# yuliakot/snark-verifier-axiom

Hardware: AMD Instinct MI355X
Metric: BN254 G1 MSM points/sec at 2^20 + KZG pairings/sec; 1/2/4/8 GPU (higher is better)
Workload: dtype u32 (254-bit Montgomery field: bucket chain 9x29-bit limbs, elsewhere 8x32-bit)

## Files before the change

### snark-verifier-axiom_amd/csrc/curve29.hpp

```cpp
#pragma once
#include "field29.hpp"

namespace sv {
namespace r29 {

struct Xyzz {
  F X, Y, ZZ, ZZZ;
};

SV29_HD F one() {
  F r;
  constexpr uint32_t O[L] = {0x157ccc21u, 0x141c2758u, 0x185230d3u, 0x14c0419u, 0xaa36fb9u,
                             0x1d4240ceu, 0x11d54c07u, 0x52ac7a8u,  0x00dc836u};
#pragma unroll
  for (int i = 0; i < L; i++) r.v[i] = O[i];
  return r;
}
SV29_HD Xyzz identity() { return {zero(), zero(), zero(), zero()}; }
SV29_HD bool is_identity(const Xyzz& p) { return is_zero(p.ZZ); }

SV29_HD Xyzz madd(const Xyzz& p, const F& x2, const F& y2, bool neg) {
  if (is_identity(p)) return {x2, neg ? sub<2>(zero(), y2) : y2, one(), one()};
  F Pd = sub<8>(mul(x2, p.ZZ), p.X);
  F Rd = sub_sgn<4>(mul(y2, p.ZZZ), neg, p.Y);
  F X = p.X, Y = p.Y, ZZ = p.ZZ, ZZZ = p.ZZZ;
  bool dbl = false;
  if (is_zero_mod_p_10p(Pd)) {
    if (!is_zero_mod_p_6p(Rd)) return identity();
    const F x2s = sqr(x2), ys = neg ? sub<2>(zero(), y2) : y2;
    Pd = add(ys, ys);
    Rd = add(add(x2s, x2s), x2s);
    X = x2, Y = ys, ZZ = one(), ZZZ = one();
    dbl = true;
  }
  const F PP = sqr(Pd), PPP = mul(Pd, PP), Q = mul(X, PP), R2 = sqr(Rd);
  const F X3 = sub_2c<6>(R2, dbl ? zero() : PPP, Q);
  const F Y3 = mul_sum2(Rd, sub<8>(Q, X3), Y, sub<2>(zero(), PPP));
  return {X3, Y3, mul(ZZ, PP), mul(ZZZ, PPP)};
}
SV29_HD Xyzz madd(const Xyzz& p, const F& x2, const F& y2) { return madd(p, x2, y2, false); }

SV29_HD F neg_one() {
  F r;
  constexpr uint32_t O[L] = {0x3003126u, 0xce8395eu, 0x420727bu, 0x1891eb7u, 0xae269bfu,
                             0x598fff2u, 0xed19539u, 0x9315e8bu, 0x229c18u};
#pragma unroll
  for (int i = 0; i < L; i++) r.v[i] = O[i];
  return r;
}
SV29_HD Xyzz start(const F& x2, const F& y2, bool neg) { return {x2, y2, one(), neg ? neg_one() : one()}; }
SV29_HD Xyzz madd_live(const Xyzz& p, const F& x2, const F& y2, bool neg, int& special) {
  const F Pd = mul_sub<8>(x2, p.ZZ, p.X);
  const F Rd = sub_sgn<4>(mul(y2, p.ZZZ), neg, p.Y);
  if (is_zero_mod_p_10p(Pd)) special = is_zero_mod_p_6p(Rd) ? 2 : 1;
  const F PP = sqr(Pd), PPP = mul(Pd, PP), Q = mul(p.X, PP);
  const F X3 = sqr_sub2c<6>(Rd, PPP, Q);
  const F Y3 = mul_sum2(Rd, sub<8>(Q, X3), p.Y, sub<2>(zero(), PPP));
  return {X3, Y3, mul(p.ZZ, PP), mul(p.ZZZ, PPP)};
}
SV29_HD Xyzz dbl_start(const F& x2, const F& y2, bool neg) {
  const F ys = neg ? sub<2>(zero(), y2) : y2;
  const F x2s = sqr(x2);
  const F Pd = add(ys, ys);
  const F Rd = add(add(x2s, x2s), x2s);
  const F PP = sqr(Pd), PPP = mul(Pd, PP), Q = mul(x2, PP);
  const F X3 = sqr_sub2c<6>(Rd, zero(), Q);
  const F Y3 = mul_sum2(Rd, sub<8>(Q, X3), ys, sub<2>(zero(), PPP));
  return {X3, Y3, PP, PPP};
}

template <bool kX4>
SV29_HD Xyzz add_t(const Xyzz& p, const Xyzz& q) {
  if (is_identity(p)) {
    if constexpr (kX4) return {csub<4>(q.X), q.Y, q.ZZ, q.ZZZ};
    else return q;
  }
  if (is_identity(q)) {
    if constexpr (kX4) return {csub<4>(p.X), p.Y, p.ZZ, p.ZZZ};
    else return p;
  }
  F U1 = mul(p.X, q.ZZ), S1 = mul(p.Y, q.ZZZ);
  F Pd = sub<2>(mul(q.X, p.ZZ), U1), Rd = sub<2>(mul(q.Y, p.ZZZ), S1);
  F qZZ = q.ZZ, qZZZ = q.ZZZ;
  bool dbl = false;
  if (is_zero_mod_p_6p(Pd)) {
    if (!is_zero_mod_p_6p(Rd)) return identity();
    const F x2 = sqr(p.X);
    Pd = add(p.Y, p.Y);
    Rd = add(add(x2, x2), x2);
    U1 = p.X, S1 = p.Y, qZZ = one(), qZZZ = one();
    dbl = true;
  }
  const F PP = sqr(Pd), PPP = mul(Pd, PP), Q = mul(U1, PP), R2 = sqr(Rd);
  const F X3 = csub<4>(sub<4>(dbl ? R2 : sub<2>(R2, PPP), add(Q, Q)));
  const F Y3 = mul_sum2(Rd, sub<4>(Q, X3), S1, sub<2>(zero(), PPP));
  return {X3, Y3, mul(mul(p.ZZ, qZZ), PP), mul(mul(p.ZZZ, qZZZ), PPP)};
}
SV29_HD Xyzz add(const Xyzz& p, const Xyzz& q) { return add_t<true>(p, q); }
SV29_HD Xyzz add_x8(const Xyzz& p, const Xyzz& q) { return add_t<false>(p, q); }

}
}
```

### snark-verifier-axiom_amd/csrc/field29.hpp

```cpp
#pragma once
#include <cstdint>

#if defined(__HIPCC__) || defined(__HIP__)
#include <hip/hip_runtime.h>
#define SV29_HD __host__ __device__ __forceinline__
#else
#define SV29_HD inline
#endif

namespace sv {
namespace r29 {

constexpr int L = 9;
constexpr uint32_t MASK = (1u << 29) - 1;

struct FqM29 {
  static constexpr uint32_t NP = 0x4866389u;
  SV29_HD static constexpr uint32_t kp(int k, int i) {
    constexpr uint32_t T[9][9] = {
        {0, 0, 0, 0, 0, 0, 0, 0, 0},
        {0x187cfd47u, 0x10460b6u, 0x1c72a34fu, 0x2d522d0u, 0x1585d978u, 0x2db40c0u, 0xa6e141u, 0xe5c2634u, 0x30644eu},
        {0x10f9fa8eu, 0x208c16du, 0x18e5469eu, 0x5aa45a1u, 0xb0bb2f0u, 0x5b68181u, 0x14dc282u, 0x1cb84c68u, 0x60c89cu},
        {0x976f7d5u, 0x30d2224u, 0x1557e9edu, 0x87f6872u, 0x918c68u, 0x891c242u, 0x1f4a3c3u, 0xb14729cu, 0x912cebu},
        {0x1f3f51cu, 0x41182dbu, 0x11ca8d3cu, 0xb548b43u, 0x161765e0u, 0xb6d0302u, 0x29b8504u, 0x197098d0u, 0xc19139u},
        {0x1a70f263u, 0x515e391u, 0xe3d308bu, 0xe29ae14u, 0xb9d3f58u, 0xe4843c3u, 0x3426645u, 0x7ccbf04u, 0xf1f588u},
        {0x12edefaau, 0x61a4448u, 0xaafd3dau, 0x10fed0e5u, 0x12318d0u, 0x11238484u, 0x3e94786u, 0x1628e538u, 0x12259d6u},
        {0xb6aecf1u, 0x71ea4ffu, 0x7227729u, 0x13d3f3b6u, 0x16a8f248u, 0x13fec544u, 0x49028c7u, 0x4850b6cu, 0x152be25u},
        {0x3e7ea38u, 0x82305b6u, 0x3951a78u, 0x16a91687u, 0xc2ecbc0u, 0x16da0605u, 0x5370a08u, 0x12e131a0u, 0x1832273u}};
    return T[k][i];
  }
};
struct FrM29 {
  static constexpr uint32_t NP = 0xfffffffu;
  SV29_HD static constexpr uint32_t kp(int k, int i) {
    constexpr uint32_t T[9][9] = {
        {0, 0, 0, 0, 0, 0, 0, 0, 0},
        {0x10000001u, 0x1f0fac9fu, 0xe5c2450u, 0x7d090f3u, 0x1585d283u, 0x2db40c0u, 0xa6e141u, 0xe5c2634u, 0x30644eu},
        {0x2u, 0x1e1f593fu, 0x1cb848a1u, 0xfa121e6u, 0xb0ba506u, 0x5b68181u, 0x14dc282u, 0x1cb84c68u, 0x60c89cu},
        {0x10000003u, 0x1d2f05deu, 0xb146cf2u, 0x1771b2dau, 0x917789u, 0x891c242u, 0x1f4a3c3u, 0xb14729cu, 0x912cebu},
        {0x4u, 0x1c3eb27eu, 0x19709143u, 0x1f4243cdu, 0x16174a0cu, 0xb6d0302u, 0x29b8504u, 0x197098d0u, 0xc19139u},
        {0x10000005u, 0x1b4e5f1du, 0x7ccb594u, 0x712d4c1u, 0xb9d1c90u, 0xe4843c3u, 0x3426645u, 0x7ccbf04u, 0xf1f588u},
        {0x6u, 0x1a5e0bbdu, 0x1628d9e5u, 0xee365b4u, 0x122ef13u, 0x11238484u, 0x3e94786u, 0x1628e538u, 0x12259d6u},
        {0x10000007u, 0x196db85cu, 0x484fe36u, 0x16b3f6a8u, 0x16a8c196u, 0x13fec544u, 0x49028c7u, 0x4850b6cu, 0x152be25u},
        {0x8u, 0x187d64fcu, 0x12e12287u, 0x1e84879bu, 0xc2e9419u, 0x16da0605u, 0x5370a08u, 0x12e131a0u, 0x1832273u}};
    return T[k][i];
  }
};

template <class M>
struct F29 {
  uint32_t v[L];
};
using F = F29<FqM29>;

template <class M = FqM29>
SV29_HD F29<M> zero() {
  F29<M> r;
#pragma unroll
  for (int i = 0; i < L; i++) r.v[i] = 0;
  return r;
}
template <int K, class M = FqM29>
SV29_HD F29<M> kp_f() {
  F29<M> r;
#pragma unroll
  for (int i = 0; i < L; i++) r.v[i] = M::kp(K, i);
  return r;
}

template <class M = FqM29>
SV29_HD F29<M> from_words(const uint32_t* w) {
  F29<M> r;
#pragma unroll
  for (int i = 0; i < L; i++) {
    const int bit = 29 * i, j = bit >> 5, s = bit & 31;
    uint32_t x = w[j] >> s;
    if (s > 3 && j + 1 < 8) x |= w[j + 1] << (32 - s);
    r.v[i] = x & MASK;
  }
  return r;
}
template <class M>
SV29_HD void to_words(const F29<M>& a, uint32_t* w) {
#pragma unroll
  for (int j = 0; j < 8; j++) {
    const int bit = 32 * j, i = bit / 29, s = bit % 29;
    uint32_t x = a.v[i] >> s;
    if (i + 1 < L) x |= a.v[i + 1] << (29 - s);
    if (s > 26 && i + 2 < L) x |= a.v[i + 2] << (58 - s);
    w[j] = x;
  }
}

SV29_HD uint64_t mad(uint32_t a, uint32_t b, uint64_t c) { return (uint64_t)a * b + c; }

#define SV29_REDUCE_COLUMN(k)                                          \
  {                                                                    \
    _Pragma("unroll") for (int i = 0; i < L; i++) {                    \
      const int j = (k) - i;                                           \
      if (i < (k) && j >= 1 && j < L) acc = mad(m[i], M::kp(1, j), acc); \
    }                                                                  \
    if ((k) < L) {                                                     \
      m[(k)] = ((uint32_t)acc * M::NP) & MASK;                         \
      acc = mad(m[(k)], M::kp(1, 0), acc);                             \
    } else {                                                           \
      t.v[(k) - L] = (uint32_t)acc & MASK;                             \
    }                                                                  \
    acc >>= 29;                                                        \
  }

template <class M>
SV29_HD F29<M> mul(const F29<M>& a, const F29<M>& b) {
  uint32_t m[L];
  F29<M> t;
  uint64_t acc = 0;
#pragma unroll
  for (int k = 0; k < 2 * L - 1; k++) {
#pragma unroll
    for (int i = 0; i < L; i++) {
      const int j = k - i;
      if (j >= 0 && j < L) acc = mad(a.v[i], b.v[j], acc);
    }
    SV29_REDUCE_COLUMN(k)
  }
  t.v[L - 1] = (uint32_t)acc;
  return t;
}

template <class M>
SV29_HD F29<M> sqr(const F29<M>& a) {
  uint32_t m[L], a2[L];
  F29<M> t;
#pragma unroll
  for (int i = 0; i < L; i++) a2[i] = a.v[i] << 1;
  uint64_t acc = 0;
#pragma unroll
  for (int k = 0; k < 2 * L - 1; k++) {
#pragma unroll
    for (int i = 0; i < L; i++) {
      const int j = k - i;
      if (j > i && j < L) acc = mad(a.v[i], a2[j], acc);
    }
    if ((k & 1) == 0 && k / 2 < L) acc = mad(a.v[k / 2], a.v[k / 2], acc);
    SV29_REDUCE_COLUMN(k)
  }
  t.v[L - 1] = (uint32_t)acc;
  return t;
}

template <class M>
SV29_HD F29<M> mul_sum2(const F29<M>& a0, const F29<M>& b0, const F29<M>& a1, const F29<M>& b1) {
  uint32_t m[L];
  F29<M> t;
  uint64_t acc = 0;
#pragma unroll
  for (int k = 0; k < 2 * L - 1; k++) {
#pragma unroll
    for (int i = 0; i < L; i++) {
      const int j = k - i;
      if (j >= 0 && j < L) {
        acc = mad(a0.v[i], b0.v[j], acc);
        acc = mad(a1.v[i], b1.v[j], acc);
      }
    }
    SV29_REDUCE_COLUMN(k)
  }
  t.v[L - 1] = (uint32_t)acc;
  return t;
}
template <class M>
SV29_HD F29<M> mul_sum3(const F29<M>& a0, const F29<M>& b0, const F29<M>& a1, const F29<M>& b1,
                        const F29<M>& a2, const F29<M>& b2) {
  uint32_t m[L];
  F29<M> t;
  uint64_t acc = 0;
#pragma unroll
  for (int k = 0; k < 2 * L - 1; k++) {
#pragma unroll
    for (int i = 0; i < L; i++) {
      const int j = k - i;
      if (j >= 0 && j < L) {
        acc = mad(a0.v[i], b0.v[j], acc);
        acc = mad(a1.v[i], b1.v[j], acc);
        acc = mad(a2.v[i], b2.v[j], acc);
      }
    }
    SV29_REDUCE_COLUMN(k)
  }
  t.v[L - 1] = (uint32_t)acc;
  return t;
}
template <class M>
SV29_HD F29<M> mul_add_hi(const F29<M>& a, const F29<M>& b, const uint32_t D[L]) {
  uint32_t m[L];
  F29<M> t;
  uint64_t acc = 0;
#pragma unroll
  for (int k = 0; k < 2 * L - 1; k++) {
    if (k >= L) acc += D[k - L];
#pragma unroll
    for (int i = 0; i < L; i++) {
      const int j = k - i;
      if (j >= 0 && j < L) acc = mad(a.v[i], b.v[j], acc);
    }
    SV29_REDUCE_COLUMN(k)
  }
  t.v[L - 1] = ((uint32_t)acc + D[L - 1]) & MASK;
  return t;
}
template <class M>
SV29_HD F29<M> sqr_add_hi(const F29<M>& a, const uint32_t D[L]) {
  uint32_t m[L], a2[L];
  F29<M> t;
#pragma unroll
  for (int i = 0; i < L; i++) a2[i] = a.v[i] << 1;
  uint64_t acc = 0;
#pragma unroll
  for (int k = 0; k < 2 * L - 1; k++) {
    if (k >= L) acc += D[k - L];
#pragma unroll
    for (int i = 0; i < L; i++) {
      const int j = k - i;
      if (j > i && j < L) acc = mad(a.v[i], a2[j], acc);
    }
    if ((k & 1) == 0 && k / 2 < L) acc = mad(a.v[k / 2], a.v[k / 2], acc);
    SV29_REDUCE_COLUMN(k)
  }
  t.v[L - 1] = ((uint32_t)acc + D[L - 1]) & MASK;
  return t;
}
#undef SV29_REDUCE_COLUMN

template <int K, class M>
SV29_HD F29<M> mul_sub(const F29<M>& a, const F29<M>& b, const F29<M>& c) {
  uint32_t D[L];
#pragma unroll
  for (int i = 0; i < L; i++) D[i] = (M::kp(K, i) + (1u << 29) - (i > 0 ? 1u : 0u)) - c.v[i];
  return mul_add_hi(a, b, D);
}
template <int K, class M>
SV29_HD F29<M> sqr_sub2c(const F29<M>& a, const F29<M>& b, const F29<M>& c) {
  uint32_t D[L];
#pragma unroll
  for (int i = 0; i < L; i++) D[i] = (M::kp(K, i) + (3u << 29) - (i > 0 ? 3u : 0u)) - (b.v[i] + (c.v[i] << 1));
  return sqr_add_hi(a, D);
}

template <class M>
SV29_HD F29<M> mul_ilp(const F29<M>& a, const F29<M>& b) {
  uint64_t c[2 * L - 1];
#pragma unroll
  for (int k = 0; k < 2 * L - 1; k++) c[k] = 0;
#pragma unroll
  for (int i = 0; i < L; i++)
#pragma unroll
    for (int j = 0; j < L; j++) c[i + j] = mad(a.v[i], b.v[j], c[i + j]);
#pragma unroll
  for (int k = 0; k < L; k++) {
    const uint32_t m = ((uint32_t)c[k] * M::NP) & MASK;
    c[k] = mad(m, M::kp(1, 0), c[k]);
    c[k + 1] += c[k] >> 29;
#pragma unroll
    for (int j = 1; j < L; j++) c[k + j] = mad(m, M::kp(1, j), c[k + j]);
  }
  F29<M> t;
  uint64_t carry = 0;
#pragma unroll
  for (int i = 0; i < L - 1; i++) {
    const uint64_t x = c[L + i] + carry;
    t.v[i] = (uint32_t)x & MASK;
    carry = x >> 29;
  }
  t.v[L - 1] = (uint32_t)carry;
  return t;
}

template <int K, class M>
SV29_HD F29<M> sub(const F29<M>& a, const F29<M>& b) {
  F29<M> r;
  int32_t c = 0;
#pragma unroll
  for (int i = 0; i < L; i++) {
    const int32_t x = (int32_t)(a.v[i] + M::kp(K, i)) - (int32_t)b.v[i] + c;
    c = x >> 29;
    r.v[i] = (uint32_t)x & MASK;
  }
  return r;
}

template <class M>
SV29_HD F29<M> add(const F29<M>& a, const F29<M>& b) {
  F29<M> r;
  uint32_t c = 0;
#pragma unroll
  for (int i = 0; i < L; i++) {
    const uint32_t x = a.v[i] + b.v[i] + c;
    c = x >> 29;
    r.v[i] = x & MASK;
  }
  return r;
}

template <int K, class M>
SV29_HD F29<M> sub_2c(const F29<M>& a, const F29<M>& b, const F29<M>& c) {
  F29<M> r;
  int32_t cy = 0;
#pragma unroll
  for (int i = 0; i < L; i++) {
    const int32_t x = (int32_t)(a.v[i] + M::kp(K, i)) - (int32_t)b.v[i] - 2 * (int32_t)c.v[i] + cy;
    cy = x >> 29;
    r.v[i] = (uint32_t)x & MASK;
  }
  return r;
}

template <int K, class M>
SV29_HD F29<M> sub_sgn(const F29<M>& a, bool neg, const F29<M>& b) {
  F29<M> r;
  int32_t cy = 0;
  const uint32_t sgn = neg ? 0xffffffffu : 1u;
#pragma unroll
  for (int i = 0; i < L; i++) {
    const int32_t x = (int32_t)(a.v[i] * sgn) + (int32_t)M::kp(K, i) - (int32_t)b.v[i] + cy;
    cy = x >> 29;
    r.v[i] = (uint32_t)x & MASK;
  }
  return r;
}

template <int K, class M>
SV29_HD F29<M> csub(const F29<M>& a) {
  F29<M> d;
  int32_t c = 0;
#pragma unroll
  for (int i = 0; i < L; i++) {
    const int32_t x = (int32_t)a.v[i] - (int32_t)M::kp(K, i) + c;
    c = x >> 29;
    d.v[i] = (uint32_t)x & MASK;
  }
  return c < 0 ? a : d;
}

template <class M>
SV29_HD bool eq(const F29<M>& a, const F29<M>& b) {
  uint32_t x = 0;
#pragma unroll
  for (int i = 0; i < L; i++) x |= a.v[i] ^ b.v[i];
  return x == 0;
}
template <class M>
SV29_HD bool is_zero(const F29<M>& a) {
  uint32_t x = 0;
#pragma unroll
  for (int i = 0; i < L; i++) x |= a.v[i];
  return x == 0;
}

SV29_HD bool is_zero_mod_p_16p(const F& a) {
  constexpr float kInvPTop = 3.1531752142655023e-07f;
  const uint32_t k = (uint32_t)((float)a.v[L - 1] * kInvPTop + 0.5f);
  if (a.v[0] != ((k * FqM29::kp(1, 0)) & MASK)) return false;
  return is_zero(csub<1>(csub<2>(csub<4>(csub<8>(a)))));
}
SV29_HD bool is_zero_mod_p_6p(const F& a) { return is_zero_mod_p_16p(a); }
SV29_HD bool is_zero_mod_p_10p(const F& a) { return is_zero_mod_p_16p(a); }

template <class M = FqM29>
SV29_HD F29<M> to_r29(const uint32_t* w) {
  F29<M> r;
#pragma unroll
  for (int i = 0; i < L; i++) {
    if (i == 0) {
      r.v[0] = (w[0] << 5) & MASK;
      continue;
    }
    const int bit = 29 * i - 5, j = bit >> 5, s = bit & 31;
    uint32_t x = w[j] >> s;
    if (s > 3 && j + 1 < 8) x |= w[j + 1] << (32 - s);
    r.v[i] = x & MASK;
  }
  const uint32_t q = (uint32_t)(((uint64_t)r.v[L - 1] * (0xffffffffull / (M::kp(1, L - 1) + 1))) >> 32);
  int64_t c = 0;
#pragma unroll
  for (int i = 0; i < L; i++) {
    const int64_t x = (int64_t)r.v[i] - (int64_t)q * M::kp(1, i) + c;
    c = x >> 29;
    r.v[i] = (uint32_t)x & MASK;
  }
  return csub<2>(r);
}
template <class M>
SV29_HD void to_r32(const F29<M>& a, uint32_t* w) {
  const uint32_t m = (a.v[0] * M::NP) & 31;
  F29<M> t;
  uint64_t c = 0;
#pragma unroll
  for (int i = 0; i < L; i++) {
    c += (uint64_t)m * M::kp(1, i) + a.v[i];
    t.v[i] = (uint32_t)c & MASK;
    c >>= 29;
  }
  F29<M> d;
#pragma unroll
  for (int i = 0; i < L; i++) d.v[i] = (t.v[i] >> 5) | ((i + 1 < L ? t.v[i + 1] : (uint32_t)c) << 24 & MASK);
  to_words(csub<1>(d), w);
}

}
}
```

### snark-verifier-axiom_amd/csrc/msm.hip

```cpp
#include <hip/hip_runtime.h>

#include <algorithm>
#include <chrono>
#include <cmath>
#include <cstdio>
#include <cstdlib>
#include <cstring>
#include <atomic>
#include <functional>
#include <string>
#include <thread>
#include <type_traits>
#include <vector>

#include "curve.hpp"
#include "curve29.hpp"
#include "glv.hpp"
#include "host_ec.hpp"
#include "msm.hpp"
#include "msm_batch.hpp"
#include "quad.hpp"
#include "runtime.hpp"

namespace sv {
// ... 120 lines not shown
  reinterpret_cast<uint4*>(out + i)[1] = make_uint4(r.x.v[4], r.x.v[5], r.x.v[6], r.x.v[7]);
  reinterpret_cast<uint4*>(out + i)[2] = make_uint4(r.y.v[0], r.y.v[1], r.y.v[2], r.y.v[3]);
  reinterpret_cast<uint4*>(out + i)[3] = make_uint4(r.y.v[4], r.y.v[5], r.y.v[6], r.y.v[7]);
}

template <int C, int NB>
__host__ __device__ constexpr int num_windows() { return (NB + C - 1) / C; }
template <int C, int NB = 255, class F>
__device__ __forceinline__ void for_each_digit(const Fr& s, F&& f) {
  constexpr int W = num_windows<C, NB>();
  uint32_t carry = 0;
  const uint32_t half = 1u << (C - 1);
  const uint32_t mask = (1u << C) - 1;
#pragma unroll
  for (int w = 0; w < W; w++) {
    const int pos = w * C;
    const int limb = pos >> 5, off = pos & 31;
    const uint32_t lo = limb < 8 ? s.v[limb] : 0;
    const uint32_t hi = (limb + 1) < 8 ? s.v[limb + 1] : 0;
    uint32_t bits = off ? ((lo >> off) | (hi << (32 - off))) : lo;
    bits = (bits & mask) + carry;
    if (bits > half) {
      f(w, (1u << C) - bits, 1u);
      carry = 1;
    } else {
      f(w, bits, 0u);
      carry = 0;
    }
  }
}

__device__ __forceinline__ Fr scalar_in(const uint4 q0, const uint4 q1, int mont_in, uint32_t* __restrict__ err) {
  Fr s;
  s.v[0] = q0.x; s.v[1] = q0.y; s.v[2] = q0.z; s.v[3] = q0.w;
  s.v[4] = q1.x; s.v[5] = q1.y; s.v[6] = q1.z; s.v[7] = q1.w;
  if (err && !s.is_reduced()) atomicOr(err, 2u);
  return mont_in ? fe_from_mont(s) : s;
}
__device__ __forceinline__ Fr load_scalar(const Fr* __restrict__ scalars, uint32_t i, int mont_in,
                                          uint32_t* __restrict__ err) {
  const uint4* p = reinterpret_cast<const uint4*>(scalars + i);
  const uint4 q0 = p[0], q1 = p[1];
  Fr s;
  s.v[0] = q0.x; s.v[1] = q0.y; s.v[2] = q0.z; s.v[3] = q0.w;
  s.v[4] = q1.x; s.v[5] = q1.y; s.v[6] = q1.z; s.v[7] = q1.w;
  if (err && !s.is_reduced()) atomicOr(err, 2u);
  return mont_in ? fe_from_mont(s) : s;
}

template <int C, bool GLV>
struct Digits {
  static constexpr int NB = GLV ? 128 : 255;
  static constexpr int W = num_windows<C, NB>();
  static constexpr int EP = GLV ? 2 * W : W;
  uint32_t h[GLV ? 2 : 1][GLV ? 4 : 8];
  uint32_t sgn[GLV ? 2 : 1];
  __device__ __forceinline__ void load(const Fr* __restrict__ scalars, uint32_t i, int mont_in,
                                       uint32_t* __restrict__ err) {
    from(load_scalar(scalars, i, mont_in, err));
  }
  __device__ __forceinline__ void from(const Fr& s) {
    if constexpr (GLV) {
      uint32_t h1[4], h2[4];
      glv_split(s.v, h1, h2);
#pragma unroll
      for (int k = 0; k < 4; k++) h[0][k] = h1[k], h[1][k] = h2[k];
#pragma unroll
      for (int q = 0; q < 2; q++) {
        sgn[q] = h[q][3] >> 31;
        h[q][3] &= 0x7fffffffu;
      }
    } else {
#pragma unroll
      for (int k = 0; k < 8; k++) h[0][k] = s.v[k];
      sgn[0] = 0;
    }
  }
  __device__ __forceinline__ void store(uint4* __restrict__ hv, uint32_t i) const {
    if constexpr (GLV) {
      hv[2 * i] = make_uint4(h[0][0], h[0][1], h[0][2], h[0][3] | (sgn[0] << 31));
      hv[2 * i + 1] = make_uint4(h[1][0], h[1][1], h[1][2], h[1][3] | (sgn[1] << 31));
    } else {
      hv[2 * i] = make_uint4(h[0][0], h[0][1], h[0][2], h[0][3]);
      hv[2 * i + 1] = make_uint4(h[0][4], h[0][5], h[0][6], h[0][7]);
    }
  }
  __device__ __forceinline__ void load_stored(const uint4* __restrict__ hv, uint32_t i) {
    const uint4 a = hv[2 * i], b = hv[2 * i + 1];
    if constexpr (GLV) {
      h[0][0] = a.x; h[0][1] = a.y; h[0][2] = a.z; h[0][3] = a.w & 0x7fffffffu;
      h[1][0] = b.x; h[1][1] = b.y; h[1][2] = b.z; h[1][3] = b.w & 0x7fffffffu;
      sgn[0] = a.w >> 31;
      sgn[1] = b.w >> 31;
    } else {
      h[0][0] = a.x; h[0][1] = a.y; h[0][2] = a.z; h[0][3] = a.w;
      h[0][4] = b.x; h[0][5] = b.y; h[0][6] = b.z; h[0][7] = b.w;
      sgn[0] = 0;
    }
  }
  template <class F>
  __device__ __forceinline__ void each(F&& f) const {
#pragma unroll
    for (int q = 0; q < (GLV ? 2 : 1); q++) {
      Fr s;
      if constexpr (GLV) {
#pragma unroll
        for (int k = 0; k < 4; k++) s.v[k] = h[q][k], s.v[4 + k] = 0u;
      } else {
#pragma unroll
        for (int k = 0; k < 8; k++) s.v[k] = h[0][k];
      }
      const uint32_t sg = sgn[q];
      for_each_digit<C, NB>(s, [&](int w, uint32_t mag, uint32_t neg) { f(w, mag, neg ^ sg, (uint32_t)q); });
    }
  }
};

__device__ __forceinline__ void glv_phix(const G1Aff* __restrict__ bases, uint32_t i, uint4* __restrict__ phix,
                                         int phi64, uint32_t* __restrict__ err) {
  const uint4* b = reinterpret_cast<const uint4*>(bases + i);
  Fq x, beta;
  const uint4 x0 = b[0], x1 = b[1];
  x.v[0] = x0.x; x.v[1] = x0.y; x.v[2] = x0.z; x.v[3] = x0.w;
  x.v[4] = x1.x; x.v[5] = x1.y; x.v[6] = x1.z; x.v[7] = x1.w;
#pragma unroll
  for (int j = 0; j < 8; j++) beta.v[j] = GLV_BETA_MONT[j];
  const Fq bx = x * beta;
  uint4* o = phix + (phi64 ? 4 : 2) * i;
  o[0] = make_uint4(bx.v[0], bx.v[1], bx.v[2], bx.v[3]);
  o[1] = make_uint4(bx.v[4], bx.v[5], bx.v[6], bx.v[7]);
  if (phi64 || err) {
    const uint4 y0 = b[2], y1 = b[3];
    if (phi64) {
      o[2] = y0;
      o[3] = y1;
    }
    if (err) {
      Fq y;
      y.v[0] = y0.x; y.v[1] = y0.y; y.v[2] = y0.z; y.v[3] = y0.w;
      y.v[4] = y1.x; y.v[5] = y1.y; y.v[6] = y1.z; y.v[7] = y1.w;
      if (!x.is_reduced() || !y.is_reduced()) atomicOr(err, 1u);
    }
  }
}

__global__ void k_glv_phix(const G1Aff* __restrict__ bases, uint32_t n, uint4* __restrict__ phix, int phi64,
                           uint32_t* __restrict__ err) {
  const uint32_t i = blockIdx.x * blockDim.x + threadIdx.x;
  if (i < n) glv_phix(bases, i, phix, phi64, err);
}

static constexpr int kPhiVtab = 2;
static constexpr int kVtabRec = 9;
__device__ __forceinline__ void st_rec29(uint2* o, const r29::F& x, const r29::F& y) {
  o[0] = make_uint2(x.v[0], x.v[1]);
  o[1] = make_uint2(x.v[2], x.v[3]);
  o[2] = make_uint2(x.v[4], x.v[5]);
  o[3] = make_uint2(x.v[6], x.v[7]);
  o[4] = make_uint2(x.v[8], y.v[0]);
  o[5] = make_uint2(y.v[1], y.v[2]);
  o[6] = make_uint2(y.v[3], y.v[4]);
  o[7] = make_uint2(y.v[5], y.v[6]);
  o[8] = make_uint2(y.v[7], y.v[8]);
}
__device__ __forceinline__ void ld_rec29(const uint2* __restrict__ o, r29::F& x, r29::F& y) {
  uint2 q[kVtabRec];
#pragma unroll
  for (int k = 0; k < kVtabRec; k++) q[k] = o[k];
  x.v[0] = q[0].x, x.v[1] = q[0].y, x.v[2] = q[1].x, x.v[3] = q[1].y, x.v[4] = q[2].x, x.v[5] = q[2].y;
  x.v[6] = q[3].x, x.v[7] = q[3].y, x.v[8] = q[4].x;
  y.v[0] = q[4].y, y.v[1] = q[5].x, y.v[2] = q[5].y, y.v[3] = q[6].x, y.v[4] = q[6].y, y.v[5] = q[7].x;
  y.v[6] = q[7].y, y.v[7] = q[8].x, y.v[8] = q[8].y;
}
__device__ __forceinline__ void vtab_put_pt(const G1Aff& a, uint32_t i, uint4* __restrict__ vtab, uint32_t nsplit,
                                            bool glv, uint32_t* __restrict__ err) {
  if (err && (!a.x.is_reduced() || !a.y.is_reduced())) atomicOr(err, 1u);
  const r29::F y = r29::to_r29(a.y.v), x = r29::to_r29(a.x.v);
  uint2* t = reinterpret_cast<uint2*>(vtab);
  st_rec29(t + kVtabRec * (size_t)i, x, y);
  if (glv) {
    constexpr uint32_t kBeta29[r29::L] = {0xa337995u, 0x158d1d23u, 0x189c9b98u, 0x12fa4e45u, 0x185faadcu,
                                         0x176f16du, 0xeed93bau,  0x14291140u, 0xc0afeu};
    r29::F beta;
#pragma unroll
    for (int j = 0; j < r29::L; j++) beta.v[j] = kBeta29[j];
    st_rec29(t + kVtabRec * ((size_t)nsplit + i), r29::mul(x, beta), y);
  }
}
__device__ __forceinline__ void vtab_put(const G1Aff* __restrict__ bases, uint32_t i, uint4* __restrict__ vtab,
                                         uint32_t nsplit, bool glv, uint32_t* __restrict__ err) {
  vtab_put_pt(load_aff(bases, i), i, vtab, nsplit, glv, err);
}
__global__ void k_vtab(const G1Aff* __restrict__ bases, uint32_t n, uint4* __restrict__ vtab, int glv,
                       uint32_t* __restrict__ err) {
  const uint32_t i = blockIdx.x * blockDim.x + threadIdx.x;
  if (i < n) vtab_put(bases, i, vtab, n, glv != 0, err);
}

__global__ void __launch_bounds__(kBlock) k_resident_prepare(const G1Aff* in, G1Aff* out, uint32_t n, int mont_in,
                                                             uint4* __restrict__ vtab, uint32_t* __restrict__ err) {
  const uint32_t i = blockIdx.x * blockDim.x + threadIdx.x;
  if (i >= n) return;
  G1Aff a;
  {
    const uint4* p = reinterpret_cast<const uint4*>(in + i);
    const uint4 q0 = p[0], q1 = p[1], q2 = p[2], q3 = p[3];
    a.x.v[0] = q0.x; a.x.v[1] = q0.y; a.x.v[2] = q0.z; a.x.v[3] = q0.w;
    a.x.v[4] = q1.x; a.x.v[5] = q1.y; a.x.v[6] = q1.z; a.x.v[7] = q1.w;
    a.y.v[0] = q2.x; a.y.v[1] = q2.y; a.y.v[2] = q2.z; a.y.v[3] = q2.w;
    a.y.v[4] = q3.x; a.y.v[5] = q3.y; a.y.v[6] = q3.z; a.y.v[7] = q3.w;
  }
  if (!a.x.is_reduced() || !a.y.is_reduced()) {
    atomicOr(err, 1u);
    a.x = Fq::zero();
    a.y = Fq::zero();
  }
  if (!mont_in && !a.is_identity()) {
    a.x = fe_to_mont(a.x);
    a.y = fe_to_mont(a.y);
  }
  uint4* o = reinterpret_cast<uint4*>(out + i);
  o[0] = make_uint4(a.x.v[0], a.x.v[1], a.x.v[2], a.x.v[3]);
  o[1] = make_uint4(a.x.v[4], a.x.v[5], a.x.v[6], a.x.v[7]);
  o[2] = make_uint4(a.y.v[0], a.y.v[1], a.y.v[2], a.y.v[3]);
  o[3] = make_uint4(a.y.v[4], a.y.v[5], a.y.v[6], a.y.v[7]);
  vtab_put_pt(a, i, vtab, n, true, nullptr);
}

__global__ void k_check_bases(const G1Aff* __restrict__ bases, uint32_t n, uint32_t* __restrict__ err) {
  const uint32_t i = blockIdx.x * blockDim.x + threadIdx.x;
  if (i >= n) return;
  const G1Aff a = load_aff(bases, i);
  if (!a.x.is_reduced() || !a.y.is_reduced()) atomicOr(err, 1u);
}

__host__ __device__ constexpr int ceil_log2(int x) { return x <= 1 ? 0 : 1 + ceil_log2((x + 1) / 2); }

template <int N>
__device__ __forceinline__ uint32_t block_excl_scan(uint32_t* x, uint32_t* part) {
  constexpr int PER = (N + kBlock - 1) / kBlock;
  const int tid = threadIdx.x;
  uint32_t loc[PER];
  uint32_t sum = 0;
#pragma unroll
  for (int j = 0; j < PER; j++) {
    const int k = tid * PER + j;
    loc[j] = k < N ? x[k] : 0u;
    sum += loc[j];
  }
  part[tid] = sum;
  __syncthreads();
  for (int off = 1; off < kBlock; off <<= 1) {
    const uint32_t u = tid >= off ? part[tid - off] : 0u;
    __syncthreads();
    part[tid] += u;
    __syncthreads();
  }
  uint32_t run = part[tid] - sum;
  const uint32_t total = part[kBlock - 1];
#pragma unroll
  for (int j = 0; j < PER; j++) {
    const int k = tid * PER + j;
    if (k < N) x[k] = run;
    run += loc[j];
  }
  __syncthreads();
  return total;
}

__device__ __forceinline__ uint32_t pack_entry32(uint32_t fine, uint32_t neg, uint32_t pt, uint32_t fb) {
  return (fb ? fine << (32 - fb) : 0u) | (neg << (31 - fb)) | pt;
}
__device__ __forceinline__ uint64_t load_entry(const uint64_t* __restrict__ tmp, uint32_t i, int e32, uint32_t fb) {
  if (!e32) return tmp[i];
  const uint32_t v = reinterpret_cast<const uint32_t*>(tmp)[i];
  const uint32_t fine = fb ? v >> (32 - fb) : 0u, neg = (v >> (31 - fb)) & 1u, pt = v & ((1u << (31 - fb)) - 1u);
  return ((uint64_t)fine << 32) | pt | (neg << 31);
}

__device__ __forceinline__ uint32_t sort_block(uint32_t b, uint32_t n, int xcd) {
  const uint32_t nfull = n & ~7u;
  if (!xcd || b >= nfull) return b;
  return (b & 7u) * (nfull >> 3) + (b >> 3);
}

template <int C, bool GLV>
__global__ void __launch_bounds__(kBlock) k_bin_hist(const Fr* __restrict__ scalars, uint32_t n, int mont_in,
                                                     uint32_t nblk, uint32_t* __restrict__ bcnt,
                                                     uint32_t* __restrict__ err, const G1Aff* __restrict__ bases,
                                                     uint4* __restrict__ phix, int phi64, int check_bases,
                                                     int xcd, int bm, uint32_t w0, uint32_t nw,
                                                     uint4* __restrict__ stored, int pf) {
  using D = Digits<C, GLV>;
  constexpr int W = D::W, LOGB = C - 1;
  constexpr int CB = coarse_bits(C, D::NB), FB = LOGB - CB, NBIN = 1 << CB;
  const uint32_t nk = nw * NBIN;
  __shared__ uint32_t h[W * NBIN];
  for (int k = threadIdx.x; k < W * NBIN; k += kBlock) h[k] = 0;
  __syncthreads();
  constexpr uint32_t CH = sort_chunk(D::EP);
  const uint32_t blk = sort_block(blockIdx.x, gridDim.x, xcd);
  const uint32_t lo = blk * CH, hi = min(n, lo + CH);
  auto count = [&](const D& d) {
    d.each([&](int w, uint32_t mag, uint32_t, uint32_t) {
      if (mag && (uint32_t)w - w0 < nw) atomicAdd(&h[(w - w0) * NBIN + ((mag - 1) >> FB)], 1u);
    });
  };
  if (phix && phi64 == kPhiVtab && pf) {
    uint32_t i = lo + threadIdx.x;
    const uint4* sp = reinterpret_cast<const uint4*>(scalars);
    const uint4* bp = reinterpret_cast<const uint4*>(bases);
    uint4 s0{}, s1{}, b0{}, b1{}, b2{}, b3{};
    if (i < hi) {
      s0 = sp[2 * (size_t)i], s1 = sp[2 * (size_t)i + 1];
      b0 = bp[4 * (size_t)i], b1 = bp[4 * (size_t)i + 1], b2 = bp[4 * (size_t)i + 2], b3 = bp[4 * (size_t)i + 3];
    }
    for (; i < hi; i += kBlock) {
      G1Aff a;
      a.x.v[0] = b0.x; a.x.v[1] = b0.y; a.x.v[2] = b0.z; a.x.v[3] = b0.w;
      a.x.v[4] = b1.x; a.x.v[5] = b1.y; a.x.v[6] = b1.z; a.x.v[7] = b1.w;
      a.y.v[0] = b2.x; a.y.v[1] = b2.y; a.y.v[2] = b2.z; a.y.v[3] = b2.w;
      a.y.v[4] = b3.x; a.y.v[5] = b3.y; a.y.v[6] = b3.z; a.y.v[7] = b3.w;
      const uint4 c0 = s0, c1 = s1;
      const uint32_t j = i + kBlock;
      if (j < hi) {
        s0 = sp[2 * (size_t)j], s1 = sp[2 * (size_t)j + 1];
        b0 = bp[4 * (size_t)j], b1 = bp[4 * (size_t)j + 1], b2 = bp[4 * (size_t)j + 2], b3 = bp[4 * (size_t)j + 3];
      }
      vtab_put_pt(a, i, phix, n, GLV, check_bases ? err : nullptr);
      D d;
// ... 270 lines not shown
    }
    __syncthreads();
    if (tid == 0) {
      uint32_t run = 0;
      for (uint32_t w = 0; w < NF; w += 64) {
        const uint32_t last = min(NF, w + 64) - 1;
        const uint32_t tot = ls[last] + lc[last];
        out[kFineCap - 8 + (w >> 6)] = run;
        run += tot;
      }
    }
    __syncthreads();
    uint32_t base_f = 0;
    if (tid < NF) base_f = ls[tid] + out[kFineCap - 8 + (tid >> 6)];
    __syncthreads();
    if (tid < NF) {
      ls[tid] = base_f;
      lc[tid] = base_f;
    }
    __syncthreads();
#pragma unroll
    for (uint32_t r = 0; r < kChunkR; r++)
      if (tid + r * 1024 < clen) out[atomicAdd(&lc[(uint32_t)(x[r] >> 32)], 1u)] = (uint32_t)x[r];
    __syncthreads();
    for (uint32_t f = tid >> 4; f < NF; f += 64) {
      const uint32_t st = ls[f], cnt = lc[f] - st, dst = fc[f];
      for (uint32_t j = tid & 15; j < cnt; j += 16) ent[dst + j] = out[st + j];
    }
    __syncthreads();
    if (tid < NF) fc[tid] += lc[tid] - ls[tid];
    __syncthreads();
  }
}


template <int MODE>
__global__ void __launch_bounds__(1024) k_fine_sort(const uint64_t* __restrict__ tmp, int e32,
                                                    const uint32_t* __restrict__ bstart, uint32_t FB, uint32_t K,
                                                    uint32_t* __restrict__ gst, uint32_t* __restrict__ tstart,
                                                    uint32_t* __restrict__ ent) {
  extern __shared__ __attribute__((aligned(16))) uint32_t fine_lds[];
  const uint32_t wb = MODE == 2 ? gridDim.x - 1 - blockIdx.x : blockIdx.x;
  const uint32_t s0 = bstart[wb], s1 = bstart[wb + 1];
  const bool big = s1 - s0 > kFineCap;
  if (MODE != 1 && !big) fine_region<true>(tmp, e32, wb, s0, s1, FB, K, gst, tstart, ent, fine_lds);
  if (MODE != 0 && big) fine_region<false>(tmp, e32, wb, s0, s1, FB, K, gst, tstart, ent, fine_lds);
}

static constexpr uint32_t kFixSerial = 8;
__device__ __forceinline__ bool join_in_block(uint32_t gs, uint32_t ge, uint32_t K) {
  const uint32_t t0 = gs / K, t1 = (ge - 1) / K;
  return t1 == t0 + 1 && t0 / kBlock == t1 / kBlock;
}
#ifndef SV_ACC_MADD32
#define SV_ACC_MADD32 xyzz_madd_2p_u
#endif
template <bool R29>
struct AccChain;
template <>
struct AccChain<false> {
  using T = G1Xyzz;
  __device__ static T identity() { return G1Xyzz::identity(); }
  __device__ static T in(const G1Xyzz& a) { return a; }
  __device__ static G1Xyzz out(const T& a) { return xyzz_canon2p(a); }
  __device__ static T madd(const T& acc, const G1Aff& p, bool neg) {
    return SV_ACC_MADD32(acc, p.x, neg ? -p.y : p.y);
  }
};
template <>
struct AccChain<true> {
  using T = r29::Xyzz;
  __device__ static T identity() { return r29::identity(); }
  __device__ static T in(const G1Xyzz& a) {
    return {r29::from_words(a.X.v), r29::from_words(a.Y.v), r29::from_words(a.ZZ.v), r29::from_words(a.ZZZ.v)};
  }
  __device__ static G1Xyzz out(const T& a) {
    G1Xyzz r;
    r29::to_words(r29::csub<4>(a.X), r.X.v);
    r29::to_words(a.Y, r.Y.v);
    r29::to_words(a.ZZ, r.ZZ.v);
    r29::to_words(a.ZZZ, r.ZZZ.v);
    return r;
  }
  __device__ static G1Xyzz canonical(const T& a) {
    G1Xyzz r;
    r29::to_r32(r29::csub<4>(a.X), r.X.v);
    r29::to_r32(a.Y, r.Y.v);
    r29::to_r32(a.ZZ, r.ZZ.v);
    r29::to_r32(a.ZZZ, r.ZZZ.v);
    return r;
  }
  __device__ static T madd(const T& acc, const G1Aff& p, bool neg) {
    const r29::F x = r29::from_words(p.x.v), y = r29::from_words(p.y.v);
    return r29::madd(acc, x, y, neg);
  }
};

#ifndef SV_ACC_MIN_BLOCKS
#define SV_ACC_MIN_BLOCKS 1
#endif
#ifndef SV_ACC29_MIN_BLOCKS
#define SV_ACC29_MIN_BLOCKS 4
#endif
template <bool ADD, bool R29, int PF = SV_ACC_PREFETCH, bool NL = R29>
__global__ void __launch_bounds__(kBlock, R29 ? SV_ACC29_MIN_BLOCKS : SV_ACC_MIN_BLOCKS) k_accumulate(
    const G1Aff* __restrict__ bases, const uint32_t* __restrict__ ent, const uint32_t* __restrict__ gst,
    const uint32_t* __restrict__ tstart, uint32_t nbt, uint32_t K, uint32_t T,
    G1Xyzz* __restrict__ bsum, G1Xyzz* __restrict__ pfirst, G1Xyzz* __restrict__ plast,
    uint32_t* __restrict__ multi, uint32_t* __restrict__ nmulti, uint32_t* __restrict__ heavy,
    uint32_t* __restrict__ nheavy, const uint4* __restrict__ phix, uint32_t nsplit, int phi64) {
  using A = AccChain<R29>;
  __shared__ G1Xyzz shead[R29 ? 1 : kBlock];
  __shared__ uint4 shead29[R29 ? 9 * kBlock : 1];
  const uint32_t t = blockIdx.x * blockDim.x + threadIdx.x;
  const uint32_t m = gst[nbt];
  const uint32_t s0 = t * K;
  const bool active = t < T && s0 < m;
  bool owner = false;
  uint32_t g = 0, gs = 0, ge = 0;
  G1Xyzz sum;
  typename A::T acc = A::identity();
  if (active) {
    const uint32_t e_end = min(s0 + K, m);
    g = tstart[t];
    gs = gst[g];
    ge = gst[g + 1];
    uint32_t seg_start = s0;
    bool first = true;
    bool empty = true;
    if constexpr (ADD) {
      if (s0 == gs) {
        if constexpr (R29) {
          acc = ld_rec29(bsum, g);
          empty = r29::is_zero(acc.ZZ);
        } else {
          acc = A::in(load_xyzz(bsum, g));
        }
      }
    }
    uint32_t vnext = 0;
    if constexpr (PF >= 1) vnext = ent[s0];
    G1Aff pnext;
    if constexpr (PF >= 2) pnext = load_vpoint(bases, phix, vnext & 0x7fffffffu, nsplit, phi64);
    if constexpr (NL) {
      static_assert(R29 && PF == 1, "the restructured loop is the 29-bit chain's");
      (void)bases;
      (void)nsplit;
      (void)phi64;
      for (uint32_t e = s0; e < e_end; e++) {
        const uint32_t v = vnext;
        if (e + 1 < e_end) vnext = ent[e + 1];
        r29::F x, y;
        ld_rec29(reinterpret_cast<const uint2*>(phix) + (size_t)kVtabRec * (v & 0x7fffffffu), x, y);
        const bool live = !(r29::is_zero(x) && r29::is_zero(y)), neg = (v & 0x80000000u) != 0;
        bool fresh = false;
        if (e >= ge || empty) {
          if (e >= ge) {
            if (seg_start == gs) {
              st_rec29(bsum, g, acc);
            } else {
              if (join_in_block(gs, ge, K)) st_rec29(reinterpret_cast<G1Xyzz*>(shead29), threadIdx.x, acc);
              else st_rec29(pfirst, t, acc);
            }
            first = false;
            do {
              g++;
              gs = ge;
              ge = gst[g + 1];
            } while (ge <= e);
            seg_start = e;
            empty = true;
            if constexpr (ADD) {
              acc = ld_rec29(bsum, g);
              empty = r29::is_zero(acc.ZZ);
            } else {
              acc.ZZ = r29::zero();
            }
          }
          if (empty && live) {
            acc = r29::start(x, y, neg);
            empty = false;
            fresh = true;
          }
        }
        if (live && !fresh) {
          int special = 0;
          acc = r29::madd_live(acc, x, y, neg, special);
          if (special) {
            if (special == 2) {
              acc = r29::dbl_start(x, y, neg);
            } else {
              acc.ZZ = r29::zero();
              empty = true;
            }
          }
        }
      }
    } else
    for (uint32_t e = s0; e < e_end; e++) {
      if (e >= ge) {
        const G1Xyzz sum = A::out(acc);
        if (seg_start == gs) {
          store_xyzz(bsum, g, sum);
        } else {
          if (join_in_block(gs, ge, K)) shead[threadIdx.x] = sum;
          else store_xyzz(pfirst, t, sum);
        }
        first = false;
        do {
          g++;
          gs = ge;
          ge = gst[g + 1];
        } while (ge <= e);
        seg_start = e;
        if constexpr (ADD) acc = A::in(load_xyzz(bsum, g));
        else acc = A::identity();
      }
      uint32_t v;
      G1Aff p;
      if constexpr (PF == 0) {
        v = ent[e];
        p = load_vpoint(bases, phix, v & 0x7fffffffu, nsplit, phi64);
      } else if constexpr (PF == 1) {
        v = vnext;
        if (e + 1 < e_end) vnext = ent[e + 1];
        p = load_vpoint(bases, phix, v & 0x7fffffffu, nsplit, phi64);
      } else {
        v = vnext;
        p = pnext;
        if (e + 1 < e_end) {
          vnext = ent[e + 1];
          pnext = load_vpoint(bases, phix, vnext & 0x7fffffffu, nsplit, phi64);
        }
      }
      if (!p.is_identity()) acc = A::madd(acc, p, (v & 0x80000000u) != 0);
    }
    if constexpr (!R29) sum = A::out(acc);
    if (seg_start == gs && e_end == ge) {
      if constexpr (R29) st_rec29(bsum, g, acc);
      else store_xyzz(bsum, g, sum);
    } else if (seg_start != gs) {
      if constexpr (R29) {
        if (join_in_block(gs, ge, K)) st_rec29(reinterpret_cast<G1Xyzz*>(shead29), threadIdx.x, acc);
        else st_rec29(pfirst, t, acc);
      } else {
        if (join_in_block(gs, ge, K)) shead[threadIdx.x] = sum;
        else store_xyzz(pfirst, t, sum);
      }
    } else if (join_in_block(gs, ge, K)) {
      owner = true;
    } else {
      if constexpr (R29) st_rec29(first ? pfirst : plast, t, acc);
      else store_xyzz(first ? pfirst : plast, t, sum);
      multi[atomicAdd(nmulti, 1u)] = g;
      if ((ge - 1) / K - gs / K > kFixSerial) heavy[atomicAdd(nheavy, 1u)] = g;
    }
  }
  __syncthreads();
  if (owner) {
    if constexpr (R29)
      st_rec29(bsum, g, r29::add_x8(acc, ld_rec29(reinterpret_cast<const G1Xyzz*>(shead29), threadIdx.x + 1)));
    else
      store_xyzz(bsum, g, xyzz_add(sum, shead[threadIdx.x + 1]));
  }
}

__device__ __forceinline__ G1Xyzz fixup_head(const G1Xyzz* __restrict__ pfirst, const G1Xyzz* __restrict__ plast,
                                             uint32_t s, uint32_t t0, uint32_t K, int r29w) {
  return load_bucket((s == t0 * K) ? pfirst : plast, t0, r29w);
}

__global__ void __launch_bounds__(kBlock) k_fixup(const uint32_t* __restrict__ gst, uint32_t K,
                                                  const G1Xyzz* __restrict__ pfirst,
                                                  const G1Xyzz* __restrict__ plast,
                                                  const uint32_t* __restrict__ multi,
                                                  const uint32_t* __restrict__ nmulti,
                                                  const uint32_t* __restrict__ heavy,
                                                  const uint32_t* __restrict__ nheavy, uint32_t gm,
                                                  G1Xyzz* __restrict__ bsum, int r29w) {
  __shared__ G1Xyzz sh[kBlock];
  const uint32_t tid = threadIdx.x;
  if (blockIdx.x < gm) {
    const uint32_t nm = *nmulti;
    const int c = tid & 3;
    for (uint32_t h = (blockIdx.x * blockDim.x + tid) >> 2; h < nm; h += (gm * blockDim.x) >> 2) {
      const uint32_t g = multi[h];
      const uint32_t s = gst[g], e = gst[g + 1];
      const uint32_t t0 = s / K, t1 = (e - 1) / K;
      if (t1 - t0 > kFixSerial) continue;
      const G1Xyzz* h0 = s == t0 * K ? pfirst : plast;
      Fq acc = r29w ? rec29_coord_canonical(rec_at(h0, t0, 1), c) : quad::ld(h0 + t0, c);
      for (uint32_t t = t0 + 1; t <= t1; t++) {
        const Fq v = r29w ? rec29_coord_canonical(rec_at(pfirst, t, 1), c) : quad::ld(pfirst + t, c);
        acc = quad::add_2p(acc, v, c);
      }
      acc = fe_canon2p(acc);
      if (r29w) rec29_coord_store(rec_at(bsum, g, 1), c, acc);
      else quad::st(bsum + g, c, acc);
    }
    return;
  }
  const uint32_t nh = *nheavy, gh = gridDim.x - gm;
  for (uint32_t h = blockIdx.x - gm; h < nh; h += gh) {
    const uint32_t g = heavy[h];
    const uint32_t s = gst[g], e = gst[g + 1];
    const uint32_t t0 = s / K, t1 = (e - 1) / K;
    G1Xyzz acc = G1Xyzz::identity();
// ... 1095 lines not shown
```

Before: 650.3 million.

## Use lazy subtraction, precomputed-inverse Montgomery columns, and vtab identity flag

The 29-bit Montgomery reduction changes so that the first seven columns take precomputed ri constants directly instead of computing a per-limb quotient and folding in kp(1,j). This removes a multiply and dependency per early column. Two subtractions feeding mul_sum2 in the bucket-add paths become carry-free lazy subtractions. The vtab now marks identity points with a high bit in the last y limb, so the hot loop tests one bit instead of two full zero checks. The risks are the bound and correctness of the new reduction and lazy outputs, and the new tag colliding with valid limb values.

```diff
diff --git a/snark-verifier-axiom_amd/csrc/curve29.hpp b/snark-verifier-axiom_amd/csrc/curve29.hpp
--- a/snark-verifier-axiom_amd/csrc/curve29.hpp
+++ b/snark-verifier-axiom_amd/csrc/curve29.hpp
@@ -55,7 +55,7 @@
   if (is_zero_mod_p_10p(Pd)) special = is_zero_mod_p_6p(Rd) ? 2 : 1;
   const F PP = sqr(Pd), PPP = mul(Pd, PP), Q = mul(p.X, PP);
   const F X3 = sqr_sub2c<6>(Rd, PPP, Q);
-  const F Y3 = mul_sum2(Rd, sub<8>(Q, X3), p.Y, sub<2>(zero(), PPP));
+  const F Y3 = mul_sum2(Rd, sub_lazy<8>(Q, X3), p.Y, sub_lazy<2>(zero(), PPP));
   return {X3, Y3, mul(p.ZZ, PP), mul(p.ZZZ, PPP)};
 }
 SV29_HD Xyzz dbl_start(const F& x2, const F& y2, bool neg) {
@@ -65,7 +65,7 @@
   const F Rd = add(add(x2s, x2s), x2s);
   const F PP = sqr(Pd), PPP = mul(Pd, PP), Q = mul(x2, PP);
   const F X3 = sqr_sub2c<6>(Rd, zero(), Q);
-  const F Y3 = mul_sum2(Rd, sub<8>(Q, X3), ys, sub<2>(zero(), PPP));
+  const F Y3 = mul_sum2(Rd, sub_lazy<8>(Q, X3), ys, sub_lazy<2>(zero(), PPP));
   return {X3, Y3, PP, PPP};
 }
 
diff --git a/snark-verifier-axiom_amd/csrc/field29.hpp b/snark-verifier-axiom_amd/csrc/field29.hpp
--- a/snark-verifier-axiom_amd/csrc/field29.hpp
+++ b/snark-verifier-axiom_amd/csrc/field29.hpp
@@ -16,6 +16,11 @@
 
 struct FqM29 {
   static constexpr uint32_t NP = 0x4866389u;
+  SV29_HD static constexpr uint32_t ri(int i) {
+    constexpr uint32_t C[9] = {0x17789a9fu, 0x5ffc3dcu,  0xd6bde42u, 0x1cf152e3u, 0x18eb055fu,
+                               0xed815e2u,  0x16626d2u, 0xb8bab0fu, 0x6d7c4u};
+    return C[i];
+  }
   SV29_HD static constexpr uint32_t kp(int k, int i) {
     constexpr uint32_t T[9][9] = {
         {0, 0, 0, 0, 0, 0, 0, 0, 0},
@@ -32,6 +37,11 @@
 };
 struct FrM29 {
   static constexpr uint32_t NP = 0xfffffffu;
+  SV29_HD static constexpr uint32_t ri(int i) {
+    constexpr uint32_t C[9] = {0x18f05361u, 0x12bb1feu,  0xf5d8135u,  0x1e6275f6u, 0x7e7a880u,
+                               0x10c6bf1fu, 0x11f74a6cu, 0x6fdaecbu, 0x183227u};
+    return C[i];
+  }
   SV29_HD static constexpr uint32_t kp(int k, int i) {
     constexpr uint32_t T[9][9] = {
         {0, 0, 0, 0, 0, 0, 0, 0, 0},
@@ -94,19 +104,26 @@
 
 SV29_HD uint64_t mad(uint32_t a, uint32_t b, uint64_t c) { return (uint64_t)a * b + c; }
 
-#define SV29_REDUCE_COLUMN(k)                                          \
-  {                                                                    \
-    _Pragma("unroll") for (int i = 0; i < L; i++) {                    \
-      const int j = (k) - i;                                           \
-      if (i < (k) && j >= 1 && j < L) acc = mad(m[i], M::kp(1, j), acc); \
-    }                                                                  \
-    if ((k) < L) {                                                     \
-      m[(k)] = ((uint32_t)acc * M::NP) & MASK;                         \
-      acc = mad(m[(k)], M::kp(1, 0), acc);                             \
-    } else {                                                           \
-      t.v[(k) - L] = (uint32_t)acc & MASK;                             \
-    }                                                                  \
-    acc >>= 29;                                                        \
+constexpr int LZ = L - 2;
+#define SV29_REDUCE_COLUMN(k)                                              \
+  {                                                                        \
+    _Pragma("unroll") for (int i = 0; i < L; i++) {                        \
+      const int j = i < LZ ? (k) - 1 - i : (k) - i;                        \
+      if (i < LZ) {                                                        \
+        if (i < (k) && j >= 0 && j < L) acc = mad(m[i], M::ri(j), acc);    \
+      } else {                                                             \
+        if (i < (k) && j >= 1 && j < L) acc = mad(m[i], M::kp(1, j), acc); \
+      }                                                                    \
+    }                                                                      \
+    if ((k) < LZ) {                                                        \
+      m[(k)] = (uint32_t)acc & MASK;                                       \
+    } else if ((k) < L) {                                                  \
+      m[(k)] = ((uint32_t)acc * M::NP) & MASK;                             \
+      acc = mad(m[(k)], M::kp(1, 0), acc);                                 \
+    } else {                                                               \
+      t.v[(k) - L] = (uint32_t)acc & MASK;                                 \
+    }                                                                      \
+    acc >>= 29;                                                            \
   }
 
 template <class M>
@@ -288,6 +305,15 @@
   return r;
 }
 
+template <int K, class M>
+SV29_HD F29<M> sub_lazy(const F29<M>& a, const F29<M>& b) {
+  F29<M> r;
+#pragma unroll
+  for (int i = 0; i < L; i++)
+    r.v[i] = a.v[i] + (M::kp(K, i) + (i < L - 1 ? 1u << 29 : 0u) - (i > 0 ? 1u : 0u)) - b.v[i];
+  return r;
+}
+
 template <class M>
 SV29_HD F29<M> add(const F29<M>& a, const F29<M>& b) {
   F29<M> r;
diff --git a/snark-verifier-axiom_amd/csrc/msm.hip b/snark-verifier-axiom_amd/csrc/msm.hip
--- a/snark-verifier-axiom_amd/csrc/msm.hip
+++ b/snark-verifier-axiom_amd/csrc/msm.hip
@@ -296,6 +296,7 @@
 
 static constexpr int kPhiVtab = 2;
 static constexpr int kVtabRec = 9;
+static constexpr uint32_t kVtabIdentity = 0x80000000u;
 __device__ __forceinline__ void st_rec29(uint2* o, const r29::F& x, const r29::F& y) {
   o[0] = make_uint2(x.v[0], x.v[1]);
   o[1] = make_uint2(x.v[2], x.v[3]);
@@ -319,7 +320,9 @@
 __device__ __forceinline__ void vtab_put_pt(const G1Aff& a, uint32_t i, uint4* __restrict__ vtab, uint32_t nsplit,
                                             bool glv, uint32_t* __restrict__ err) {
   if (err && (!a.x.is_reduced() || !a.y.is_reduced())) atomicOr(err, 1u);
-  const r29::F y = r29::to_r29(a.y.v), x = r29::to_r29(a.x.v);
+  r29::F y = r29::to_r29(a.y.v);
+  const r29::F x = r29::to_r29(a.x.v);
+  if (r29::is_zero(x) && r29::is_zero(y)) y.v[r29::L - 1] = kVtabIdentity;
   uint2* t = reinterpret_cast<uint2*>(vtab);
   st_rec29(t + kVtabRec * (size_t)i, x, y);
   if (glv) {
@@ -896,7 +899,7 @@
         if (e + 1 < e_end) vnext = ent[e + 1];
         r29::F x, y;
         ld_rec29(reinterpret_cast<const uint2*>(phix) + (size_t)kVtabRec * (v & 0x7fffffffu), x, y);
-        const bool live = !(r29::is_zero(x) && r29::is_zero(y)), neg = (v & 0x80000000u) != 0;
+        const bool live = (y.v[r29::L - 1] & kVtabIdentity) == 0, neg = (v & 0x80000000u) != 0;
         bool fresh = false;
         if (e >= ge || empty) {
           if (e >= ge) {
```

Measured after the change: 668.2 million, median of 6. 2.7% higher.
